# 23skdu/longbow

Measured on AMD Instinct MI355X. Metric: k-NN queries/sec (batch=1024, k=100), 1Mx768 f32, higher is better.
Workload: dtype f32

## Files before the change

### longbow_amd/csrc/kernels_gemm.hip

```cpp
#include "lb_admit.h"

#include <cstdlib>

namespace lb {

constexpr int BM = 128;
constexpr int BN = 128;
constexpr int BK = 32;
constexpr int GEMM_THREADS = 256;

struct GemmArgs {
    const float *X;
    const float *norm2;
    const float *rnorm;
    int64_t row_begin, row_end;
    int D;
    const float *Q;
    int nq;
    const uint8_t *mask;
    const uint32_t *rowmap;
    CandState cs;
    int n_row_tiles, n_q_tiles;
    int boot;
};

__device__ __forceinline__ int swz_off(int row, int chunk)
{
    return row * BK + ((chunk ^ ((row >> 1) & 7)) << 2);
}

template <int MODE>
__device__ __forceinline__ f32x4 load_chunk(const float *base, int64_t row, int D, int k)
{
    f32x4 v = {0.f, 0.f, 0.f, 0.f};
    const float *p = base + row * (int64_t)D + k;
    if (MODE == 2) {
        v = *reinterpret_cast<const f32x4 *>(p);
    } else if (MODE == 1) {
        if (k < D) v = *reinterpret_cast<const f32x4 *>(p);
    } else {
        if (k + 0 < D) v.x = p[0];
        if (k + 1 < D) v.y = p[1];
        if (k + 2 < D) v.z = p[2];
        if (k + 3 < D) v.w = p[3];
    }
    return v;
}

template <int METRIC, int ALIGNED>
__global__ __launch_bounds__(GEMM_THREADS, 2) void gemm_filter_kernel(GemmArgs a)
{
    constexpr bool GLDS = ALIGNED == 2;
    const int b = blockIdx.x;
    const int xcd = b & 7;
    const int in_xcd = b >> 3;
    const int qt = in_xcd % a.n_q_tiles;
    const int rt = (in_xcd / a.n_q_tiles) * 8 + xcd;
    if (rt >= a.n_row_tiles) return;

    __shared__ __attribute__((aligned(16))) float lds_all[2 * 2 * BM * BK + BM + BM + BM / 4];
    float(*lds)[2][BM * BK] = reinterpret_cast<float(*)[2][BM * BK]>(lds_all);
    float *s_aux = lds_all + 2 * 2 * BM * BK;
    uint32_t *s_rowid = reinterpret_cast<uint32_t *>(s_aux + BM);
    uint8_t *s_vis = reinterpret_cast<uint8_t *>(s_rowid + BM);

    const int tid = threadIdx.x;
    const int lane = tid & 63;
    const int wave = tid >> 6;
    const int wr = wave >> 1, wc = wave & 1;
    const int l31 = lane & 31, h = lane >> 5;

    const int64_t row0 = a.row_begin + (int64_t)rt * BM;
    const int q0 = qt * BN;
    const int64_t last_row = a.row_end - 1;
    const int last_q = a.nq - 1;

    auto corpus_row = [&](int64_t pos) -> int64_t {
        if (pos > last_row) pos = last_row;
        return a.rowmap ? (int64_t)a.rowmap[pos] : pos;
    };
    const int64_t side_ri = corpus_row(row0 + (tid & (BM - 1)));

    int st_row[4], st_ch[4];
    int64_t st_xrow[4];
    int st_qrow[4];
#pragma unroll
    for (int i = 0; i < 4; i++) {
        int c = tid + GEMM_THREADS * i;
        st_row[i] = c >> 3;
        st_ch[i] = c & 7;
        st_xrow[i] = corpus_row(row0 + st_row[i]);
        int qr = q0 + st_row[i];
        st_qrow[i] = qr < last_q ? qr : last_q;
    }

    f32x16 acc[2][2];
#pragma unroll
    for (int i = 0; i < 2; i++)
#pragma unroll
        for (int j = 0; j < 2; j++)
#pragma unroll
            for (int r = 0; r < 16; r++) acc[i][j][r] = 0.f;

    const int nk = (a.D + BK - 1) / BK;
    f32x4 ra[4], rb[4];

    const float *gsrcA[4], *gsrcB[4];
    if (GLDS) {
#pragma unroll
        for (int i = 0; i < 4; i++) {
            const int j = wave * 4 + i;
            const int row = j * 8 + (lane >> 3);
            const int c = (lane & 7) ^ ((row >> 1) & 7);
            const int64_t xr = corpus_row(row0 + row);
            int qr = q0 + row;
            if (qr > last_q) qr = last_q;
            gsrcA[i] = a.X + xr * (int64_t)a.D + 4 * c;
            gsrcB[i] = a.Q + (int64_t)qr * a.D + 4 * c;
        }
    }
    const int wave_u = __builtin_amdgcn_readfirstlane(wave);
    auto glds_piece = [&](int p, int stage, int k0) {
        const int i = p >> 1;
        const int j = wave_u * 4 + i;
        if ((p & 1) == 0)
            __builtin_amdgcn_global_load_lds(
                (const __attribute__((address_space(1))) void *)(gsrcA[i] + k0),
                (__attribute__((address_space(3))) void *)(&lds[stage][0][j * 8 * BK]), 16, 0,
                2);
        else
            __builtin_amdgcn_global_load_lds(
                (const __attribute__((address_space(1))) void *)(gsrcB[i] + k0),
                (__attribute__((address_space(3))) void *)(&lds[stage][1][j * 8 * BK]), 16, 0, 0);
    };
    auto glds_stage = [&](int stage, int k0) {
#pragma unroll
        for (int p = 0; p < 8; p++) glds_piece(p, stage, k0);
    };
    if (GLDS) glds_stage(0, 0);
    const float aux_r = side_aux<METRIC>(a.norm2, a.rnorm, side_ri);
    uint8_t side_vis = 1;
    if (a.mask) side_vis = a.mask[side_ri];
    uint64_t tau_raw[2];
#pragma unroll
    for (int tn = 0; tn < 2; tn++) {
        const int qj = q0 + wc * 64 + tn * 32 + l31;
        tau_raw[tn] = lane_tau(a.cs.tau, qj, a.nq, a.boot);
    }
    if (tid < BM) {
        s_aux[tid] = aux_r;
        s_vis[tid] = (row0 + tid <= last_row && side_vis) ? (uint8_t)1 : (uint8_t)0;
        s_rowid[tid] = (uint32_t)side_ri;
    }
    float tau_key[2];
    uint32_t tau_row[2];
#pragma unroll
    for (int tn = 0; tn < 2; tn++) {
        tau_key[tn] = tau_key_of(tau_raw[tn]);
        tau_row[tn] = entry_row(tau_raw[tn]);
    }
    if (!GLDS) {
#pragma unroll
        for (int i = 0; i < 4; i++) {
            ra[i] = load_chunk<ALIGNED>(a.X, st_xrow[i], a.D, st_ch[i] * 4);
            rb[i] = load_chunk<ALIGNED>(a.Q, st_qrow[i], a.D, st_ch[i] * 4);
        }
#pragma unroll
        for (int i = 0; i < 4; i++) {
            *reinterpret_cast<f32x4 *>(&lds[0][0][swz_off(st_row[i], st_ch[i])]) = ra[i];
            *reinterpret_cast<f32x4 *>(&lds[0][1][swz_off(st_row[i], st_ch[i])]) = rb[i];
        }
    }
    __syncthreads();

    if constexpr (GLDS) {
        struct Frag {
            f32x4 a[2], b[2];
        };
        auto ldfrag = [&](Frag &f, int stage, int s) {
            const float *As = lds[stage][0];
            const float *Bs = lds[stage][1];
            const int ch = 2 * s + h;
#pragma unroll
            for (int t = 0; t < 2; t++) {
                f.a[t] = *reinterpret_cast<const f32x4 *>(&As[swz_off(wr * 64 + t * 32 + l31, ch)]);
                f.b[t] = *reinterpret_cast<const f32x4 *>(&Bs[swz_off(wc * 64 + t * 32 + l31, ch)]);
            }
        };
        auto mfma16 = [&](const Frag &f) {
#pragma unroll
            for (int e = 0; e < 4; e++)
#pragma unroll
                for (int tm = 0; tm < 2; tm++)
#pragma unroll
                    for (int tn = 0; tn < 2; tn++)
                        acc[tm][tn] = __builtin_amdgcn_mfma_f32_32x32x2f32(f.a[tm][e], f.b[tn][e], acc[tm][tn], 0, 0, 0);
        };
        Frag F0, F1;
        auto steps012 = [&](int cur) {
            ldfrag(F1, cur, 1);
            mfma16(F0);
            ldfrag(F0, cur, 2);
            mfma16(F1);
            ldfrag(F1, cur, 3);
            mfma16(F0);
#pragma unroll
            for (int s = 0; s < 3; s++) {
                __builtin_amdgcn_sched_group_barrier(0x008, 2, 0);
                __builtin_amdgcn_sched_group_barrier(0x100, 4, 0);
                __builtin_amdgcn_sched_group_barrier(0x008, 14, 0);
            }
            __builtin_amdgcn_sched_barrier(0);
        };
        ldfrag(F0, 0, 0);
        if (nk > 1) glds_stage(1, BK);
        int kt = 0;
        for (; kt + 2 < nk; kt++) {
            const int cur = kt & 1;
            steps012(cur);
            __syncthreads();
            const int k0 = (kt + 2) * BK;
            ldfrag(F0, cur ^ 1, 0);
#pragma unroll
            for (int p = 0; p < 8; p++) glds_piece(p, cur, k0);
            mfma16(F1);
            __builtin_amdgcn_sched_group_barrier(0x008, 2, 0);
            __builtin_amdgcn_sched_group_barrier(0x100, 4, 0);
#pragma unroll
            for (int p = 0; p < 7; p++) {
                __builtin_amdgcn_sched_group_barrier(0x020, 1, 0);
                __builtin_amdgcn_sched_group_barrier(0x008, 2, 0);
            }
            __builtin_amdgcn_sched_group_barrier(0x020, 1, 0);
        }
        if (kt + 1 < nk) {
            const int cur = kt & 1;
            steps012(cur);
            __syncthreads();
            ldfrag(F0, cur ^ 1, 0);
            mfma16(F1);
            __builtin_amdgcn_sched_group_barrier(0x008, 2, 0);
            __builtin_amdgcn_sched_group_barrier(0x100, 4, 0);
            __builtin_amdgcn_sched_group_barrier(0x008, 14, 0);
            kt++;
        }
        steps012(kt & 1);
        mfma16(F1);
    } else {
        for (int kt = 0; kt < nk; kt++) {
            const int cur = kt & 1;
            const bool has_next = kt + 1 < nk;
            if (has_next) {
                const int k0 = (kt + 1) * BK;
#pragma unroll
                for (int i = 0; i < 4; i++) {
                    ra[i] = load_chunk<ALIGNED>(a.X, st_xrow[i], a.D, k0 + st_ch[i] * 4);
                    rb[i] = load_chunk<ALIGNED>(a.Q, st_qrow[i], a.D, k0 + st_ch[i] * 4);
                }
            }
            const float *As = lds[cur][0];
            const float *Bs = lds[cur][1];
            f32x4 fa[2][2], fb[2][2];
#pragma unroll
            for (int t = 0; t < 2; t++) {
                fa[0][t] = *reinterpret_cast<const f32x4 *>(&As[swz_off(wr * 64 + t * 32 + l31, h)]);
                fb[0][t] = *reinterpret_cast<const f32x4 *>(&Bs[swz_off(wc * 64 + t * 32 + l31, h)]);
            }
#pragma unroll
            for (int s = 0; s < 4; s++) {
                const int cb = s & 1, nb = cb ^ 1;
                if (s < 3) {
                    const int ch = 2 * (s + 1) + h;
#pragma unroll
                    for (int t = 0; t < 2; t++) {
                        fa[nb][t] = *reinterpret_cast<const f32x4 *>(&As[swz_off(wr * 64 + t * 32 + l31, ch)]);
                        fb[nb][t] = *reinterpret_cast<const f32x4 *>(&Bs[swz_off(wc * 64 + t * 32 + l31, ch)]);
                    }
                }
#pragma unroll
                for (int e = 0; e < 4; e++)
#pragma unroll
                    for (int tm = 0; tm < 2; tm++)
#pragma unroll
                        for (int tn = 0; tn < 2; tn++)
                            acc[tm][tn] = __builtin_amdgcn_mfma_f32_32x32x2f32(fa[cb][tm][e], fb[cb][tn][e],
                                                                              acc[tm][tn], 0, 0, 0);
                if (s == 1 && has_next) {
                    const int nxt = cur ^ 1;
#pragma unroll
                    for (int i = 0; i < 4; i++) {
                        *reinterpret_cast<f32x4 *>(&lds[nxt][0][swz_off(st_row[i], st_ch[i])]) = ra[i];
                        *reinterpret_cast<f32x4 *>(&lds[nxt][1][swz_off(st_row[i], st_ch[i])]) = rb[i];
                    }
                }
            }
            __syncthreads();
        }
    }

    float aux[2][4][4];
    uint32_t rid[2][4][4];
    uint32_t vbits = 0;
#pragma unroll
    for (int tm = 0; tm < 2; tm++)
#pragma unroll
        for (int g = 0; g < 4; g++)
            vbits |= tile_rows4(s_aux, s_rowid, s_vis, wr * 64 + tm * 32 + 8 * g + 4 * h, aux[tm][g], rid[tm][g]) << (tm * 16 + g * 4);
#pragma unroll
    for (int tn = 0; tn < 2; tn++) {
        const int qj = q0 + wc * 64 + tn * 32 + l31;
        const bool qok = qj < a.nq;
        uint64_t *list = a.cs.lists + (size_t)(qok ? qj : 0) * a.cs.cap;
        if (a.boot) {
            if (qok) {
#pragma unroll
                for (int tm = 0; tm < 2; tm++)
#pragma unroll
                    for (int g = 0; g < 4; g++) {
                        const int64_t rbase = row0 + wr * 64 + tm * 32 + 8 * g + 4 * h;
                        uint64_t ent[4];
#pragma unroll
                        for (int e = 0; e < 4; e++)
                            ent[e] = ((vbits >> (tm * 16 + g * 4 + e)) & 1u) ? pack_entry(cand_key<METRIC>(acc[tm][tn][4 * g + e], aux[tm][g][e]), rid[tm][g][e]) : kEntryMax;
                        uint64_t *dst = list + (rbase - a.row_begin);
                        if (rbase + 3 < a.row_end) {
                            typedef unsigned long long u64x2 __attribute__((ext_vector_type(2)));
                            u64x2 v0 = {ent[0], ent[1]}, v1 = {ent[2], ent[3]};
                            *reinterpret_cast<u64x2 *>(dst) = v0;
                            *reinterpret_cast<u64x2 *>(dst + 2) = v1;
                        } else {
#pragma unroll
                            for (int e = 0; e < 4; e++)
                                if (rbase + e < a.row_end) dst[e] = ent[e];
                        }
                    }
            }
            continue;
        }
        uint32_t bits = 0;
#pragma unroll
        for (int tm = 0; tm < 2; tm++)
#pragma unroll
            for (int g = 0; g < 4; g++)
#pragma unroll
                for (int e = 0; e < 4; e++)
                    bits |= admit_exact(cand_key<METRIC>(acc[tm][tn][4 * g + e], aux[tm][g][e]), rid[tm][g][e], tau_key[tn], tau_row[tn]) << (tm * 16 + g * 4 + e);
        bits &= vbits;
        if (bits) {
            uint32_t pos = atomicAdd(&a.cs.cnt[qj], (uint32_t)__builtin_popcount(bits));
#pragma unroll
            for (int tm = 0; tm < 2; tm++)
#pragma unroll
                for (int g = 0; g < 4; g++)
#pragma unroll
                    for (int e = 0; e < 4; e++)
                        if (bits & (1u << (tm * 16 + g * 4 + e))) {
                            const uint32_t ri = rid[tm][g][e];
                            if (pos < a.cs.cap) list[pos] = pack_entry(cand_key<METRIC>(acc[tm][tn][4 * g + e], aux[tm][g][e]), ri);
                            pos++;
                        }
        }
    }
}

__global__ __launch_bounds__(256) void split_bf16_kernel(const float *src, float *dst, int64_t n8)
{
    for (int64_t i = (int64_t)blockIdx.x * blockDim.x + threadIdx.x; i < n8; i += (int64_t)gridDim.x * blockDim.x) {
        bf16x8 hi, lo;
        split_bf16x8(*reinterpret_cast<const f32x4 *>(src + i * 8), *reinterpret_cast<const f32x4 *>(src + i * 8 + 4), hi, lo);
        const int64_t grp = i >> 1;
        const int kb = (int)(i & 1);
        char *g = reinterpret_cast<char *>(dst) + grp * 64;
        *reinterpret_cast<bf16x8 *>(g + kb * 16) = hi;
        *reinterpret_cast<bf16x8 *>(g + 32 + kb * 16) = lo;
    }
}

void launch_split_bf16(const float *src, float *dst, int64_t rows, int D, hipStream_t s)
{
    const int64_t n8 = rows * (int64_t)D / 8;
    if (n8 <= 0) return;
    int64_t blocks = (n8 + 255) / 256;
    if (blocks > 16384) blocks = 16384;
    hipLaunchKernelGGL(split_bf16_kernel, dim3((unsigned)blocks), dim3(256), 0, s, src, dst, n8);
}

void launch_gemm_filter(int metric, const float *X, const float *norm2, const float *rnorm,
                        int64_t row_begin, int64_t row_end, int D, const float *Q, int nq,
                        const uint8_t *mask, const uint32_t *rowmap, CandState cs, bool boot, hipStream_t s)
{
    if (row_end <= row_begin || nq <= 0) return;
    GemmArgs a;
    a.rowmap = rowmap;
    a.boot = boot ? 1 : 0;
    a.X = X; a.norm2 = norm2; a.rnorm = rnorm;
    a.row_begin = row_begin; a.row_end = row_end; a.D = D;
    a.Q = Q; a.nq = nq; a.mask = mask; a.cs = cs;
    a.n_row_tiles = (int)((row_end - row_begin + BM - 1) / BM);
    a.n_q_tiles = (nq + BN - 1) / BN;
    const int groups = (a.n_row_tiles + 7) / 8;
    dim3 grid((unsigned)(groups * 8 * a.n_q_tiles));
    const bool aligned = (D % 4 == 0) && ((reinterpret_cast<uintptr_t>(X) & 15) == 0) &&
                         ((reinterpret_cast<uintptr_t>(Q) & 15) == 0);
    const int mode = !aligned ? 0 : (D % BK == 0 ? 2 : 1);
#define LB_GEMM(M, AL) hipLaunchKernelGGL((gemm_filter_kernel<M, AL>), grid, dim3(GEMM_THREADS), 0, s, a)
#define LB_GEMM_M(M)                 \
    do {                             \
        if (mode == 2) LB_GEMM(M, 2); \
        else if (mode == 1) LB_GEMM(M, 1); \
        else LB_GEMM(M, 0);           \
    } while (0)
    if (metric == METRIC_L2) LB_GEMM_M(METRIC_L2);
    else if (metric == METRIC_COS) LB_GEMM_M(METRIC_COS);
    else LB_GEMM_M(METRIC_DOT);
#undef LB_GEMM_M
#undef LB_GEMM
}

}
```

### longbow_amd/csrc/lb_admit.h

```cpp
#pragma once
#include "lb_device.h"

namespace lb {

template <int METRIC>
__device__ __forceinline__ float cand_key(float dot, float aux)
{
    if (METRIC == METRIC_L2) return fmaf(-2.0f, dot, aux);
    if (METRIC == METRIC_COS) return -dot * aux;
    return -dot;
}

__device__ __forceinline__ uint64_t lane_tau(const uint64_t *tau_q, int qj, int nq, bool none)
{
    uint64_t tau = none ? 0ull : tau_q[qj < nq ? qj : nq - 1];
    if (qj >= nq) tau = 0ull;
    return tau;
}
template <int METRIC>
__device__ __forceinline__ float side_aux(const float *norm2, const float *rnorm, int64_t ri)
{
    return METRIC == METRIC_L2 ? norm2[ri] : (METRIC == METRIC_COS ? rnorm[ri] : 0.f);
}
__device__ __forceinline__ uint32_t tile_rows4(const float *s_aux, const uint32_t *s_rowid, const uint8_t *s_vis, int lr,
                                               float (&aux)[4], uint32_t (&rid)[4])
{
    const f32x4 av = *reinterpret_cast<const f32x4 *>(&s_aux[lr]);
    const uint4 rv = *reinterpret_cast<const uint4 *>(&s_rowid[lr]);
    const uint32_t vv = *reinterpret_cast<const uint32_t *>(&s_vis[lr]);
    aux[0] = av.x; aux[1] = av.y; aux[2] = av.z; aux[3] = av.w;
    rid[0] = rv.x; rid[1] = rv.y; rid[2] = rv.z; rid[3] = rv.w;
    return (vv & 1u) | ((vv >> 7) & 2u) | ((vv >> 14) & 4u) | ((vv >> 21) & 8u);
}

__device__ __forceinline__ uint32_t admit_exact(float key, uint32_t ri, float tk, uint32_t tr)
{
    return (uint32_t)(key < tk) | ((uint32_t)(key == tk) & (uint32_t)(ri < tr));
}
template <int FL_CAP, int NQ, int NTHREADS>
struct LocalList {
    static constexpr int CAP = FL_CAP;
    uint32_t *cnt;
    uint32_t *qcnt;
    uint32_t *qbase;
    uint64_t *ent;
    uint16_t *q;
    uint16_t *rk;
    __device__ __forceinline__ LocalList(uint32_t *counters, uint64_t *entries)
        : cnt(counters), qcnt(counters + 1), qbase(counters + 1 + NQ), ent(entries),
          q(reinterpret_cast<uint16_t *>(entries + FL_CAP)), rk(reinterpret_cast<uint16_t *>(entries + FL_CAP) + FL_CAP)
    {
    }
    __device__ __forceinline__ void reset(int tid) const
    {
        if (tid == 0) *cnt = 0;
        if (tid < NQ) qcnt[tid] = 0;
    }
    __device__ __forceinline__ void reserved_unused(uint32_t lp, uint32_t n) const
    {
        for (uint32_t i = lp; i < lp + n && i < (uint32_t)FL_CAP; i++) ent[i] = kEntryMax;
    }
    __device__ __forceinline__ void flush(int tid, CandState cs, int q0) const
    {
        __syncthreads();
        if (tid < NQ) {
            const uint32_t n = qcnt[tid];
            qbase[tid] = n ? atomicAdd(&cs.cnt[q0 + tid], n) : 0u;
        }
        __syncthreads();
        const uint32_t total = *cnt < (uint32_t)FL_CAP ? *cnt : (uint32_t)FL_CAP;
        for (uint32_t i = tid; i < total; i += NTHREADS) {
            const uint64_t e = ent[i];
            if (e == kEntryMax) continue;
            const int ql = (int)q[i];
            const uint32_t pos = qbase[ql] + (uint32_t)rk[i];
            if (pos < cs.cap) cs.lists[(size_t)(q0 + ql) * cs.cap + pos] = e;
        }
    }
};

}
```

Measured before the change: 87250.

## Overlap side-data loads with final MFMAs and batch admission atomics per wave

Moves the LDS loads of per-row aux, row ids and visibility bits so they are issued during the final MFMA block, using sched_group_barrier to interleave them. The admission epilogue now computes masks for both query columns first, issues both atomics up front, and uses a DPP wave-wide OR so the scatter loop only visits bit positions some lane admitted. This aims to hide LDS and atomic latency and cut the unrolled predicated scatter work in the non-boot epilogue, at the cost of more live registers and a manual waitcnt that must be correct.

```diff
diff --git a/longbow_amd/csrc/kernels_gemm.hip b/longbow_amd/csrc/kernels_gemm.hip
--- a/longbow_amd/csrc/kernels_gemm.hip
+++ b/longbow_amd/csrc/kernels_gemm.hip
@@ -93,6 +93,17 @@
         int qr = q0 + st_row[i];
         st_qrow[i] = qr < last_q ? qr : last_q;
     }
+
+    float aux[2][4][4];
+    uint32_t rid[2][4][4];
+    uint32_t vbits = 0;
+    auto load_side = [&]() {
+#pragma unroll
+        for (int tm = 0; tm < 2; tm++)
+#pragma unroll
+            for (int g = 0; g < 4; g++)
+                vbits |= tile_rows4(s_aux, s_rowid, s_vis, wr * 64 + tm * 32 + 8 * g + 4 * h, aux[tm][g], rid[tm][g]) << (tm * 16 + g * 4);
+    };
 
     f32x16 acc[2][2];
 #pragma unroll
@@ -245,7 +256,11 @@
             kt++;
         }
         steps012(kt & 1);
+        load_side();
         mfma16(F1);
+        __builtin_amdgcn_sched_group_barrier(0x008, 2, 0);
+        __builtin_amdgcn_sched_group_barrier(0x100, 24, 0);
+        __builtin_amdgcn_sched_group_barrier(0x008, 14, 0);
     } else {
         for (int kt = 0; kt < nk; kt++) {
             const int cur = kt & 1;
@@ -296,69 +311,80 @@
             }
             __syncthreads();
         }
-    }
-
-    float aux[2][4][4];
-    uint32_t rid[2][4][4];
-    uint32_t vbits = 0;
-#pragma unroll
-    for (int tm = 0; tm < 2; tm++)
-#pragma unroll
-        for (int g = 0; g < 4; g++)
-            vbits |= tile_rows4(s_aux, s_rowid, s_vis, wr * 64 + tm * 32 + 8 * g + 4 * h, aux[tm][g], rid[tm][g]) << (tm * 16 + g * 4);
+        load_side();
+    }
+
+    if (a.boot) {
+#pragma unroll
+        for (int tn = 0; tn < 2; tn++) {
+            const int qj = q0 + wc * 64 + tn * 32 + l31;
+            if (qj >= a.nq) continue;
+            uint64_t *list = a.cs.lists + (size_t)qj * a.cs.cap;
+#pragma unroll
+            for (int tm = 0; tm < 2; tm++)
+#pragma unroll
+                for (int g = 0; g < 4; g++) {
+                    const int64_t rbase = row0 + wr * 64 + tm * 32 + 8 * g + 4 * h;
+                    uint64_t ent[4];
+#pragma unroll
+                    for (int e = 0; e < 4; e++)
+                        ent[e] = ((vbits >> (tm * 16 + g * 4 + e)) & 1u) ? pack_entry(cand_key<METRIC>(acc[tm][tn][4 * g + e], aux[tm][g][e]), rid[tm][g][e]) : kEntryMax;
+                    uint64_t *dst = list + (rbase - a.row_begin);
+                    if (rbase + 3 < a.row_end) {
+                        typedef unsigned long long u64x2 __attribute__((ext_vector_type(2)));
+                        u64x2 v0 = {ent[0], ent[1]}, v1 = {ent[2], ent[3]};
+                        *reinterpret_cast<u64x2 *>(dst) = v0;
+                        *reinterpret_cast<u64x2 *>(dst + 2) = v1;
+                    } else {
+#pragma unroll
+                        for (int e = 0; e < 4; e++)
+                            if (rbase + e < a.row_end) dst[e] = ent[e];
+                    }
+                }
+        }
+        return;
+    }
+    uint32_t bits[2];
 #pragma unroll
     for (int tn = 0; tn < 2; tn++) {
-        const int qj = q0 + wc * 64 + tn * 32 + l31;
-        const bool qok = qj < a.nq;
-        uint64_t *list = a.cs.lists + (size_t)(qok ? qj : 0) * a.cs.cap;
-        if (a.boot) {
-            if (qok) {
-#pragma unroll
-                for (int tm = 0; tm < 2; tm++)
-#pragma unroll
-                    for (int g = 0; g < 4; g++) {
-                        const int64_t rbase = row0 + wr * 64 + tm * 32 + 8 * g + 4 * h;
-                        uint64_t ent[4];
-#pragma unroll
-                        for (int e = 0; e < 4; e++)
-                            ent[e] = ((vbits >> (tm * 16 + g * 4 + e)) & 1u) ? pack_entry(cand_key<METRIC>(acc[tm][tn][4 * g + e], aux[tm][g][e]), rid[tm][g][e]) : kEntryMax;
-                        uint64_t *dst = list + (rbase - a.row_begin);
-                        if (rbase + 3 < a.row_end) {
-                            typedef unsigned long long u64x2 __attribute__((ext_vector_type(2)));
-                            u64x2 v0 = {ent[0], ent[1]}, v1 = {ent[2], ent[3]};
-                            *reinterpret_cast<u64x2 *>(dst) = v0;
-                            *reinterpret_cast<u64x2 *>(dst + 2) = v1;
-                        } else {
-#pragma unroll
-                            for (int e = 0; e < 4; e++)
-                                if (rbase + e < a.row_end) dst[e] = ent[e];
+        uint32_t bt = 0;
+#pragma unroll
+        for (int tm = 0; tm < 2; tm++)
+#pragma unroll
+            for (int g = 0; g < 4; g++)
+#pragma unroll
+                for (int e = 0; e < 4; e++)
+                    bt |= admit_exact(cand_key<METRIC>(acc[tm][tn][4 * g + e], aux[tm][g][e]), rid[tm][g][e], tau_key[tn], tau_row[tn]) << (tm * 16 + g * 4 + e);
+        bits[tn] = bt & vbits;
+    }
+    uint32_t pos[2] = {0u, 0u};
+#pragma unroll
+    for (int tn = 0; tn < 2; tn++)
+        if (bits[tn]) pos[tn] = atomicAdd(&a.cs.cnt[q0 + wc * 64 + tn * 32 + l31], (uint32_t)__builtin_popcount(bits[tn]));
+    const uint32_t wave_bits[2] = {wave_or_u32(bits[0]), wave_or_u32(bits[1])};
+    if (wave_bits[0] | wave_bits[1]) {
+        __builtin_amdgcn_s_waitcnt(0x0f70);
+        asm volatile("" : "+v"(pos[0]), "+v"(pos[1]));
+#pragma unroll
+        for (int tn = 0; tn < 2; tn++) {
+            const int qj = q0 + wc * 64 + tn * 32 + l31;
+            uint64_t *list = a.cs.lists + (size_t)(qj < a.nq ? qj : 0) * a.cs.cap;
+            uint32_t p = pos[tn];
+#pragma unroll
+            for (int tm = 0; tm < 2; tm++)
+#pragma unroll
+                for (int g = 0; g < 4; g++)
+#pragma unroll
+                    for (int e = 0; e < 4; e++) {
+                        const uint32_t m = 1u << (tm * 16 + g * 4 + e);
+                        if (wave_bits[tn] & m) {
+                            asm volatile("");
+                            if (bits[tn] & m) {
+                                if (p < a.cs.cap) list[p] = pack_entry(cand_key<METRIC>(acc[tm][tn][4 * g + e], aux[tm][g][e]), rid[tm][g][e]);
+                                p++;
+                            }
                         }
                     }
-            }
-            continue;
-        }
-        uint32_t bits = 0;
-#pragma unroll
-        for (int tm = 0; tm < 2; tm++)
-#pragma unroll
-            for (int g = 0; g < 4; g++)
-#pragma unroll
-                for (int e = 0; e < 4; e++)
-                    bits |= admit_exact(cand_key<METRIC>(acc[tm][tn][4 * g + e], aux[tm][g][e]), rid[tm][g][e], tau_key[tn], tau_row[tn]) << (tm * 16 + g * 4 + e);
-        bits &= vbits;
-        if (bits) {
-            uint32_t pos = atomicAdd(&a.cs.cnt[qj], (uint32_t)__builtin_popcount(bits));
-#pragma unroll
-            for (int tm = 0; tm < 2; tm++)
-#pragma unroll
-                for (int g = 0; g < 4; g++)
-#pragma unroll
-                    for (int e = 0; e < 4; e++)
-                        if (bits & (1u << (tm * 16 + g * 4 + e))) {
-                            const uint32_t ri = rid[tm][g][e];
-                            if (pos < a.cs.cap) list[pos] = pack_entry(cand_key<METRIC>(acc[tm][tn][4 * g + e], aux[tm][g][e]), ri);
-                            pos++;
-                        }
         }
     }
 }
diff --git a/longbow_amd/csrc/lb_admit.h b/longbow_amd/csrc/lb_admit.h
--- a/longbow_amd/csrc/lb_admit.h
+++ b/longbow_amd/csrc/lb_admit.h
@@ -37,6 +37,22 @@
 {
     return (uint32_t)(key < tk) | ((uint32_t)(key == tk) & (uint32_t)(ri < tr));
 }
+template <int CTRL, int ROW_MASK>
+__device__ __forceinline__ uint32_t or_dpp_u32(uint32_t v)
+{
+    return v | (uint32_t)__builtin_amdgcn_update_dpp((int)v, (int)v, CTRL, ROW_MASK, 0xf, false);
+}
+__device__ __forceinline__ uint32_t wave_or_u32(uint32_t v)
+{
+    v = or_dpp_u32<0xB1, 0xf>(v);
+    v = or_dpp_u32<0x4E, 0xf>(v);
+    v = or_dpp_u32<0x141, 0xf>(v);
+    v = or_dpp_u32<0x140, 0xf>(v);
+    v = or_dpp_u32<0x142, 0xa>(v);
+    v = or_dpp_u32<0x143, 0xc>(v);
+    return (uint32_t)__builtin_amdgcn_readlane((int)v, 63);
+}
+
 template <int FL_CAP, int NQ, int NTHREADS>
 struct LocalList {
     static constexpr int CAP = FL_CAP;
```

After: 88000 (median of 6 runs). No clear change (+0.9%).

## Add 128x256 wide-query-tile GEMM filter kernel with triple-buffered LDS DMA

Applied to the files above, without the earlier changes.

Adds a new GEMM-filter kernel that processes 256 queries per block instead of 128, halving re-reads of corpus rows across query tiles. It uses a 3-stage LDS pipeline fed by global_load_lds with XOR swizzling, BK=16, 32x32x2 f32 MFMA, and explicit scheduling group barriers to interleave loads and MFMAs. The kernel is selected for aligned, non-boot launches when enough workgroups exist. In exchange it uses more accumulators and registers per thread, which may limit occupancy, and it adds a separate code path to maintain.

```diff
diff --git a/longbow_amd/csrc/kernels_gemm.hip b/longbow_amd/csrc/kernels_gemm.hip
--- a/longbow_amd/csrc/kernels_gemm.hip
+++ b/longbow_amd/csrc/kernels_gemm.hip
@@ -363,6 +363,227 @@
     }
 }
 
+constexpr int BNW = 256;
+constexpr int BKW = 16;
+constexpr int WSTAGE = (BM + BNW) * BKW;
+constexpr int WSTAGES = 3;
+
+__device__ __forceinline__ int swz16_off(int row, int chunk)
+{
+    return row * BKW + ((chunk ^ ((row >> 2) & 3)) << 2);
+}
+
+template <int METRIC>
+__global__ __launch_bounds__(GEMM_THREADS, 2) void gemm_filter_q256_kernel(GemmArgs a)
+{
+    const int b = blockIdx.x;
+    const int xcd = b & 7;
+    const int in_xcd = b >> 3;
+    const int qt = in_xcd % a.n_q_tiles;
+    const int rt = (in_xcd / a.n_q_tiles) * 8 + xcd;
+    if (rt >= a.n_row_tiles) return;
+
+    __shared__ __attribute__((aligned(16))) float lds_all[WSTAGES * WSTAGE + BM + BM + BM / 4];
+    float *s_aux = lds_all + WSTAGES * WSTAGE;
+    uint32_t *s_rowid = reinterpret_cast<uint32_t *>(s_aux + BM);
+    uint8_t *s_vis = reinterpret_cast<uint8_t *>(s_rowid + BM);
+
+    const int tid = threadIdx.x;
+    const int lane = tid & 63;
+    const int wave = tid >> 6;
+    const int wr = wave >> 1, wc = wave & 1;
+    const int l31 = lane & 31, h = lane >> 5;
+
+    const int64_t row0 = a.row_begin + (int64_t)rt * BM;
+    const int q0 = qt * BNW;
+    const int64_t last_row = a.row_end - 1;
+    const int last_q = a.nq - 1;
+
+    auto corpus_row = [&](int64_t pos) -> int64_t {
+        if (pos > last_row) pos = last_row;
+        return a.rowmap ? (int64_t)a.rowmap[pos] : pos;
+    };
+    const int64_t side_ri = corpus_row(row0 + (tid & (BM - 1)));
+
+    const float *gsrcA[2], *gsrcB[4];
+#pragma unroll
+    for (int i = 0; i < 2; i++) {
+        const int row = (wave * 2 + i) * 16 + (lane >> 2);
+        const int c = (lane & 3) ^ ((row >> 2) & 3);
+        gsrcA[i] = a.X + corpus_row(row0 + row) * (int64_t)a.D + 4 * c;
+    }
+#pragma unroll
+    for (int i = 0; i < 4; i++) {
+        const int row = (wave * 4 + i) * 16 + (lane >> 2);
+        const int c = (lane & 3) ^ ((row >> 2) & 3);
+        int qr = q0 + row;
+        if (qr > last_q) qr = last_q;
+        gsrcB[i] = a.Q + (int64_t)qr * a.D + 4 * c;
+    }
+    const int wave_u = __builtin_amdgcn_readfirstlane(wave);
+    auto glds_piece = [&](int p, int buf, int k0) {
+        float *st = lds_all + buf * WSTAGE;
+        if (p == 0 || p == 2) {
+            const int i = p >> 1;
+            __builtin_amdgcn_global_load_lds((const __attribute__((address_space(1))) void *)(gsrcA[i] + k0),
+                                             (__attribute__((address_space(3))) void *)(st + (wave_u * 2 + i) * 16 * BKW), 16, 0,
+                                             2);
+        } else {
+            const int i = p == 1 ? 0 : p - 2;
+            __builtin_amdgcn_global_load_lds((const __attribute__((address_space(1))) void *)(gsrcB[i] + k0),
+                                             (__attribute__((address_space(3))) void *)(st + BM * BKW + (wave_u * 4 + i) * 16 * BKW), 16, 0, 0);
+        }
+    };
+
+    f32x16 acc[2][4];
+#pragma unroll
+    for (int i = 0; i < 2; i++)
+#pragma unroll
+        for (int j = 0; j < 4; j++)
+#pragma unroll
+            for (int r = 0; r < 16; r++) acc[i][j][r] = 0.f;
+
+    const int nk = a.D / BKW;
+#pragma unroll
+    for (int p = 0; p < 6; p++) glds_piece(p, 0, 0);
+#pragma unroll
+    for (int p = 0; p < 6; p++) glds_piece(p, 1, BKW);
+    const float aux_r = side_aux<METRIC>(a.norm2, a.rnorm, side_ri);
+    uint8_t side_vis = 1;
+    if (a.mask) side_vis = a.mask[side_ri];
+    uint64_t tau_raw[4];
+#pragma unroll
+    for (int tn = 0; tn < 4; tn++) tau_raw[tn] = lane_tau(a.cs.tau, q0 + wc * 128 + tn * 32 + l31, a.nq, false);
+    if (tid < BM) {
+        s_aux[tid] = aux_r;
+        s_vis[tid] = (row0 + tid <= last_row && side_vis) ? (uint8_t)1 : (uint8_t)0;
+        s_rowid[tid] = (uint32_t)side_ri;
+    }
+    float tau_key[4];
+    uint32_t tau_row[4];
+#pragma unroll
+    for (int tn = 0; tn < 4; tn++) {
+        tau_key[tn] = tau_key_of(tau_raw[tn]);
+        tau_row[tn] = entry_row(tau_raw[tn]);
+    }
+    __syncthreads();
+
+    struct Frag {
+        f32x4 a[2], b[4];
+    };
+    auto ldfrag = [&](Frag &f, int buf, int s) {
+        const float *As = lds_all + buf * WSTAGE;
+        const float *Bs = As + BM * BKW;
+        const int ch = 2 * s + h;
+#pragma unroll
+        for (int t = 0; t < 2; t++) f.a[t] = *reinterpret_cast<const f32x4 *>(&As[swz16_off(wr * 64 + t * 32 + l31, ch)]);
+#pragma unroll
+        for (int t = 0; t < 4; t++) f.b[t] = *reinterpret_cast<const f32x4 *>(&Bs[swz16_off(wc * 128 + t * 32 + l31, ch)]);
+    };
+    auto mfma32 = [&](const Frag &f) {
+#pragma unroll
+        for (int e = 0; e < 4; e++)
+#pragma unroll
+            for (int tm = 0; tm < 2; tm++)
+#pragma unroll
+                for (int tn = 0; tn < 4; tn++)
+                    acc[tm][tn] = __builtin_amdgcn_mfma_f32_32x32x2f32(f.a[tm][e], f.b[tn][e], acc[tm][tn], 0, 0, 0);
+    };
+    Frag F0, F1;
+    auto kstep = [&](int cur, int nxt, int dst, int k0, bool dma, bool next) {
+        ldfrag(F1, cur, 1);
+        if (dma) {
+#pragma unroll
+            for (int p = 0; p < 6; p++) glds_piece(p, dst, k0);
+        }
+        mfma32(F0);
+        if (next) ldfrag(F0, nxt, 0);
+        mfma32(F1);
+        __builtin_amdgcn_sched_group_barrier(0x008, 8, 0);
+        __builtin_amdgcn_sched_group_barrier(0x100, 6, 0);
+        if (dma) {
+#pragma unroll
+            for (int p = 0; p < 6; p++) {
+                __builtin_amdgcn_sched_group_barrier(0x020, 1, 0);
+                __builtin_amdgcn_sched_group_barrier(0x008, 4, 0);
+            }
+        } else {
+            __builtin_amdgcn_sched_group_barrier(0x008, 24, 0);
+        }
+        __builtin_amdgcn_sched_group_barrier(0x008, 8, 0);
+        if (next) __builtin_amdgcn_sched_group_barrier(0x100, 6, 0);
+        __builtin_amdgcn_sched_group_barrier(0x008, 24, 0);
+        __builtin_amdgcn_sched_barrier(0);
+    };
+    ldfrag(F0, 0, 0);
+    int cur = 0;
+    for (int kt = 0; kt + 2 < nk; kt++) {
+        const int nxt = cur == 2 ? 0 : cur + 1;
+        const int dst = nxt == 2 ? 0 : nxt + 1;
+        kstep(cur, nxt, dst, (kt + 2) * BKW, true, true);
+        __syncthreads();
+        cur = nxt;
+    }
+    {
+        const int nxt = cur == 2 ? 0 : cur + 1;
+        kstep(cur, nxt, 0, 0, false, true);
+        kstep(nxt, 0, 0, 0, false, false);
+    }
+
+    auto half_rows = [&](int tm, float(&aux)[4][4], uint32_t(&rid)[4][4]) -> uint32_t {
+        uint32_t vb = 0;
+#pragma unroll
+        for (int g = 0; g < 4; g++) vb |= tile_rows4(s_aux, s_rowid, s_vis, wr * 64 + tm * 32 + 8 * g + 4 * h, aux[g], rid[g]) << (g * 4);
+        return vb;
+    };
+    uint32_t bits[4] = {0u, 0u, 0u, 0u};
+#pragma unroll
+    for (int tm = 0; tm < 2; tm++) {
+        float aux[4][4];
+        uint32_t rid[4][4];
+        const uint32_t vb = half_rows(tm, aux, rid);
+#pragma unroll
+        for (int tn = 0; tn < 4; tn++) {
+            uint32_t bt = 0;
+#pragma unroll
+            for (int g = 0; g < 4; g++)
+#pragma unroll
+                for (int e = 0; e < 4; e++)
+                    bt |= admit_exact(cand_key<METRIC>(acc[tm][tn][4 * g + e], aux[g][e]), rid[g][e], tau_key[tn], tau_row[tn]) << (g * 4 + e);
+            bits[tn] |= (bt & vb) << (tm * 16);
+        }
+    }
+    asm volatile("" : "+v"(bits[0]), "+v"(bits[1]), "+v"(bits[2]), "+v"(bits[3]));
+    uint32_t pos[4];
+#pragma unroll
+    for (int tn = 0; tn < 4; tn++) {
+        asm volatile("" : "=v"(pos[tn]));
+        if (bits[tn]) pos[tn] = atomicAdd(&a.cs.cnt[q0 + wc * 128 + tn * 32 + l31], (uint32_t)__builtin_popcount(bits[tn]));
+    }
+    asm volatile("" : "+v"(pos[0]), "+v"(pos[1]), "+v"(pos[2]), "+v"(pos[3]));
+#pragma unroll
+    for (int tm = 0; tm < 2; tm++) {
+        if (((bits[0] | bits[1] | bits[2] | bits[3]) >> (tm * 16)) & 0xffffu) {
+            float aux[4][4];
+            uint32_t rid[4][4];
+            half_rows(tm, aux, rid);
+#pragma unroll
+            for (int tn = 0; tn < 4; tn++) {
+                const int qj = q0 + wc * 128 + tn * 32 + l31;
+                uint64_t *list = a.cs.lists + (size_t)(qj < a.nq ? qj : 0) * a.cs.cap;
+#pragma unroll
+                for (int g = 0; g < 4; g++)
+#pragma unroll
+                    for (int e = 0; e < 4; e++)
+                        if (bits[tn] & (1u << (tm * 16 + g * 4 + e))) {
+                            if (pos[tn] < a.cs.cap) list[pos[tn]] = pack_entry(cand_key<METRIC>(acc[tm][tn][4 * g + e], aux[g][e]), rid[g][e]);
+                            pos[tn]++;
+                        }
+            }
+        }
+    }
+}
+
 __global__ __launch_bounds__(256) void split_bf16_kernel(const float *src, float *dst, int64_t n8)
 {
     for (int64_t i = (int64_t)blockIdx.x * blockDim.x + threadIdx.x; i < n8; i += (int64_t)gridDim.x * blockDim.x) {
@@ -398,11 +619,23 @@
     a.Q = Q; a.nq = nq; a.mask = mask; a.cs = cs;
     a.n_row_tiles = (int)((row_end - row_begin + BM - 1) / BM);
     a.n_q_tiles = (nq + BN - 1) / BN;
-    const int groups = (a.n_row_tiles + 7) / 8;
-    dim3 grid((unsigned)(groups * 8 * a.n_q_tiles));
     const bool aligned = (D % 4 == 0) && ((reinterpret_cast<uintptr_t>(X) & 15) == 0) &&
                          ((reinterpret_cast<uintptr_t>(Q) & 15) == 0);
     const int mode = !aligned ? 0 : (D % BK == 0 ? 2 : 1);
+    static const int wide_qtile = lb_tunable("LB_WIDE_QTILE", 0);
+    static const int q256_min_wgs = lb_tunable("LB_WIDE_Q256_MIN_WGS", 1024);
+    const int n_q256 = (nq + BNW - 1) / BNW;
+    const bool q256 = mode == 2 && !boot && wide_qtile != 128 && n_q256 * BNW == a.n_q_tiles * BN &&
+                      (int64_t)a.n_row_tiles * n_q256 >= q256_min_wgs;
+    if (q256) a.n_q_tiles = n_q256;
+    const int groups = (a.n_row_tiles + 7) / 8;
+    dim3 grid((unsigned)(groups * 8 * a.n_q_tiles));
+    if (q256) {
+        if (metric == METRIC_L2) hipLaunchKernelGGL((gemm_filter_q256_kernel<METRIC_L2>), grid, dim3(GEMM_THREADS), 0, s, a);
+        else if (metric == METRIC_COS) hipLaunchKernelGGL((gemm_filter_q256_kernel<METRIC_COS>), grid, dim3(GEMM_THREADS), 0, s, a);
+        else hipLaunchKernelGGL((gemm_filter_q256_kernel<METRIC_DOT>), grid, dim3(GEMM_THREADS), 0, s, a);
+        return;
+    }
 #define LB_GEMM(M, AL) hipLaunchKernelGGL((gemm_filter_kernel<M, AL>), grid, dim3(GEMM_THREADS), 0, s, a)
 #define LB_GEMM_M(M)                 \
     do {                             \
```

After: 87090 before, 87110 after, median of 3. About the same (+0.0%).
